# houzhijian/CONE

Measured on AMD Instinct MI355X. Metric: windows/sec + queries/sec, Ego4D-NLQ win_len=90 d=256 top-k=20, higher is better.
Workload: dtype f32

## Files before the change

cone_amd/csrc/api.hip:

```cpp
#include <stdarg.h>
#include <string.h>

#include <vector>

#include "common.h"
#include "gemm_tall.h"
#include "rows_chain.h"

namespace cone {

static thread_local char g_err[512] = "";
void set_error(const char* fmt, ...) {
    va_list ap;
    va_start(ap, fmt);
    vsnprintf(g_err, sizeof(g_err), fmt, ap);
    va_end(ap);
}

struct Linear { const float* w = nullptr; const float* b = nullptr; };
struct LNorm { const float* g = nullptr; const float* b = nullptr; };
struct Mha { const float* in_w = nullptr; const float* in_b = nullptr; Linear out; };
struct EncLayer { Mha sa; Linear l1, l2; LNorm n1, n2; };
struct DecLayer { Mha sa, ca; Linear l1, l2; LNorm n1, n2, n3; };

// ... 13 lines not shown
    const float* txt_pos_emb = nullptr; int txt_pos_rows = 0; cone::LNorm txt_pos_ln;
    int pre_norm = 0; cone::LNorm enc_norm;
    cone::Linear dec_k, dec_v;
    const float* dec_vT[CONE_MAX_LAYERS] = {};
    float* dec0_tgt1 = nullptr; float* dec0_dq = nullptr; float* dec0_scratch = nullptr;
    float* dec_sa_tab[CONE_MAX_LAYERS] = {}; float* dec_ca_tab[CONE_MAX_LAYERS] = {};
    float* tab_arena = nullptr; const float* tab_pos_rows = nullptr; const float* tab_pos_qk = nullptr; int tab_max_v_l = 0;
    int opt_dec_fold = 2;
    int opt_dec0_const = 1;
    int opt_l0_gather = 1;
    int opt_pos_tables = 1;
    int opt_gemm = 0;
    int opt_gemm_tall_min = -1;
    cone::TailWeights enc_tail[CONE_MAX_LAYERS] = {}, dec_tail[CONE_MAX_LAYERS] = {};
    char* split_img = nullptr; char* bf16_img = nullptr;
    int opt_qkv_fused = 1;
    int opt_split_bf16 = 0;
    int opt_bf16 = 0;
    int opt_res_gather = 1;
    int opt_spread = 1;
    int opt_chain = 1;
    int opt_ffn_fused = 2;
    int gen_native = 0;
    int opt_general = 0;
    int opt_general_bf16 = 0;
    char* gen_bf16_img = nullptr;
    struct GenImage { const float* W; const void* img; };
    std::vector<GenImage> gen_bf16_images;
    int opt_max_tokens = CONE_MAX_WINDOW_TOKENS;
    char* f32_img = nullptr; char* f32_tall_img = nullptr;
    struct TallImage { const float* W; int N; const char* img; };
    std::vector<TallImage> tall_images;
    int opt_tail_packed = CONE_TAIL_PACKED_DEFAULT;
    int opt_gemm_tall_packed = CONE_GEMM_TALL_PACKED_DEFAULT;
    const void* tall_image(const float* W, int N) const {
        for (const TallImage& t : tall_images) {
            const uintptr_t w = (uintptr_t)W, base = (uintptr_t)t.W;
            if (w < base || (w - base) % (32 * 256 * sizeof(float)) != 0) continue;
            const size_t off = (w - base) / sizeof(float);
            if (off / 256 + (size_t)N <= (size_t)t.N) return t.img + (size_t)(off / (32 * 256)) * cone::F32_PACK_CHUNK_BYTES;
        }
        return nullptr;
    }
    bool long_windows() const { return opt_max_tokens > CONE_MAX_WINDOW_TOKENS; }
    bool general() const { return gen_native || opt_general || long_windows(); }
};

namespace cone {

struct ArenaBuilder {
    struct Item { const float* src; size_t n; const float** dst; };
    std::vector<Item> items;
    size_t total = 0;
    void add(const float* src, size_t n, const float** dst) {
        items.push_back({src, n, dst});
        total += align_up(n, 64);
    }
};

static int dec0_constants(cone_model* m, hipStream_t s);
static int build_pos_tables(const cone_model* m, int max_v_l, float* pos_rows, float* pos_qk, hipStream_t s);
static int64_t pos_table_rows(int max_v_l) { return (int64_t)max_v_l * (max_v_l + 1) / 2 + 1; }

static void free_model(cone_model* m) {
    if (m->arena) (void)hipFree(m->arena);
    if (m->split_img) (void)hipFree(m->split_img);
// ... 576 lines not shown
                                m->nq, Lmax, s);
    const bool ride = l == 0 && p.sal_ride;
    if (ride) CONE_CHECK_HIP(hipMemsetAsync(c.saliency, 0, (size_t)c.B * c.Lv_max * sizeof(float), s));
    return launch_dec_cross_mfma(f.DQ, XP, MEM, pos, c.vlen, f.off, dl.ca.in_w + 256 * 256, m->dec_vT[l], dl.ca.in_b + 512, f.DATT,
                                 c.B, m->nq, Lmax, l == 0 && p.slabs ? f.QKS : nullptr, s, p.cross[l], ride ? m->saliency.w : nullptr,
                                 ride ? m->saliency.b : nullptr, ride ? c.saliency : nullptr, ride ? c.Lv_max : 0);
}
static AttnSrc table_attn_src(const FwdCall& c, const cone_layer0& l0, int l) {
    const size_t rows = (size_t)pos_table_rows(l0.max_v_l);
    AttnSrc src{};
    src.vlen = c.vlen; src.pos_zero_row = (int)rows - 1;
    src.pos_qk = l0.pos_qk + (size_t)l * rows * 512;
    if (l0.txt_pos_qk) { src.txt_pos_qk = l0.txt_pos_qk + (size_t)l * l0.n_txt * 512; src.trow0 = c.trow0; }
    return src;
}

static int forward_packed_prenorm(const cone_model* m, const FwdCall& c, const FwdPlan& p, FwdBuffers& f, hipStream_t s) {
    const int B = c.B, Lmax = c.Lv_max + c.Lq_max, Mmax = B * Lmax, T = B * m->nq, nd = m->n_dec, ff = m->ff;
    const int* Mdev = f.off + B;
    RUN(launch_scan_lengths(c.vlen, c.qlen, B, f.off, s));
    RUN(launch_pack_pos(c.vproj, c.vrow0, c.vlen, c.tproj, c.trow0, c.qlen, f.off, m->dim_t, f.X, f.POS, f.XP, B, Lmax, s,
                        m->txt_pos_emb, m->txt_pos_ln.g, m->txt_pos_ln.b));
    GemmArgs g;
    for (int l = 0; l < m->n_enc; ++l) {
        const EncLayer& e = m->enc[l];
        RUN(launch_layernorm(f.X, 256, e.n1.g, e.n1.b, f.X1, 256, Mmax, Mdev, 256, s));
        float* QK = f.QKV; float* V = f.QKV + (size_t)Mmax * 512;
        g = G(m, f.X1, 256, e.sa.in_w, 256, e.sa.in_b, QK, 512, Mmax, Mdev, 512, 256);
        g.A2 = f.POS; g.lda2 = 256;
        RUN(launch_gemm(g, s));
        RUN(launch_gemm(G(m, f.X1, 256, e.sa.in_w + 512 * 256, 256, e.sa.in_b + 512, V, 256, Mmax, Mdev, 256, 256), s));
        AttnSrc src{};
        src.Q = QK; src.K = QK + 256; src.V = V; src.ldq = src.ldk = 512; src.ldv = 256;
        RUN(launch_enc_attn(ATTN_PACKED, src, f.ATT, f.off, B, Lmax, s));
        g = G(m, f.ATT, 256, e.sa.out.w, 256, e.sa.out.b, f.X, 256, Mmax, Mdev, 256, 256, EPI_RESIDUAL);
        g.R = f.X; g.ldr = 256;
        RUN(launch_gemm(g, s));
        RUN(launch_layernorm(f.X, 256, e.n2.g, e.n2.b, f.X1, 256, Mmax, Mdev, 256, s));
        RUN(launch_gemm(G(m, f.X1, 256, e.l1.w, 256, e.l1.b, f.H, ff, Mmax, Mdev, ff, 256, EPI_RELU), s));
        g = G(m, f.H, ff, e.l2.w, ff, e.l2.b, f.X, 256, Mmax, Mdev, 256, ff, EPI_RESIDUAL);
        g.R = f.X; g.ldr = 256;
        RUN(launch_gemm(g, s));
    }
    RUN(launch_layernorm(f.X, 256, m->enc_norm.g, m->enc_norm.b, f.X1, 256, Mmax, Mdev, 256, s));
    const float* MEM = f.X1;
    g = G(m, MEM, 256, m->dec_k.w, 256, m->dec_k.b, f.KD, 256 * nd, Mmax, Mdev, 256 * nd, 256);
    g.A2 = f.POS; g.lda2 = 256;
    RUN(launch_gemm(g, s));
    RUN(launch_gemm(G(m, MEM, 256, m->dec_v.w, 256, m->dec_v.b, f.VD, 256 * nd, Mmax, Mdev, 256 * nd, 256), s));
    CONE_CHECK_HIP(hipMemsetAsync(f.TGT, 0, (size_t)T * 256 * sizeof(float), s));
    for (int l = 0; l < nd; ++l) {
        const DecLayer& dl = m->dec[l];
        RUN(dec_layer_front(m, f, l, B, true, s));
        RUN(dec_cross_attn(m, c, p, f, l, MEM, s));
        g = G(m, f.DATT, 256, dl.ca.out.w, 256, dl.ca.out.b, f.TGT, 256, T, nullptr, 256, 256, EPI_RESIDUAL);
        g.R = f.TGT; g.ldr = 256;
        RUN(launch_gemm(g, s));
        RUN(launch_layernorm(f.TGT, 256, dl.n3.g, dl.n3.b, f.TGT1, 256, T, nullptr, 256, s));
        RUN(launch_gemm(G(m, f.TGT1, 256, dl.l1.w, 256, dl.l1.b, f.DH, ff, T, nullptr, ff, 256, EPI_RELU), s));
        g = G(m, f.DH, ff, dl.l2.w, ff, dl.l2.b, f.TGT, 256, T, nullptr, 256, ff, EPI_RESIDUAL);
        g.R = f.TGT; g.ldr = 256;
        RUN(launch_gemm(g, s));
        RUN(launch_layernorm(f.TGT, 256, m->dec_norm.g, m->dec_norm.b, f.HS + (size_t)l * T * 256, 256, T, nullptr, 256, s));
    }
    return heads_and_taps(m, c, HeadBufs{f.HS, f.S1, f.S2, f.LG, f.SP, f.off}, MEM, false, s);
}
// ... 233 lines not shown
        RUN(launch_pack_l0(c.vproj, c.vrow0, c.vlen, c.tproj, c.trow0, c.qlen, f.off, m->dim_t, nullptr, nullptr, nullptr, f.X,
                           nullptr, nullptr, nullptr, B, Lmax, s));
    } else {
        RUN(launch_pack_pos(c.vproj, c.vrow0, c.vlen, c.tproj, c.trow0, c.qlen, f.off, m->dim_t, f.X, f.POS, f.XP, B, Lmax, s,
                            m->txt_pos_emb, m->txt_pos_ln.g, m->txt_pos_ln.b));
    }
    if (p.pre && !p.gather_res)
        RUN(launch_layernorm(f.X, 256, m->enc[0].n1.g, m->enc[0].n1.b, Z, 256, Mmax, Mdev, 256, s));

    bool qkv_fused = false;
    for (int l = 0; l < m->n_enc; ++l) {
        const EncLayer& e = m->enc[l];
        AttnSrc src{};
        int mode = ATTN_PACKED;
        if (l == 0 && p.gather0) {
            mode = ATTN_GATHER;
            src = table_attn_src(c, l0, 0);
            src.qkv_vid = l0.qkv_vid; src.qkv_txt = l0.qkv_txt; src.vrow0 = c.vrow0; src.trow0 = c.trow0;
        } else if (l == 0 && p.caches) {
            src.Q = f.QKV; src.K = f.QKV + 256; src.V = f.QKV + (size_t)Mmax * 512;
            src.ldq = src.ldk = 512; src.ldv = 256;
        } else if (p.tables) {
            if (!qkv_fused)
                RUN(encoder_qkv(m, l, p.pre ? Z : f.X, f.QKV, Mmax, Mdev, s, !p.pre));
            mode = ATTN_POSADD;
            src = table_attn_src(c, l0, l);
            src.Q = f.QKV; src.K = f.QKV + 256; src.V = f.QKV + 512; src.ldq = src.ldk = src.ldv = 768;
        } else {
            float* QK = f.QKV; float* V = f.QKV + (size_t)Mmax * 512;
            RUN(launch_gemm(G(m, f.XP, 256, e.sa.in_w, 256, e.sa.in_b, QK, 512, Mmax, Mdev, 512, 256), s));
            RUN(launch_gemm(G(m, f.X, 256, e.sa.in_w + 512 * 256, 256, e.sa.in_b + 512, V, 256, Mmax, Mdev, 256, 256), s));
            src.Q = QK; src.K = QK + 256; src.V = V; src.ldq = src.ldk = 512; src.ldv = 256;
        }
        RUN(launch_enc_attn(mode, src, f.ATT, f.off, B, Lmax, s));
        const bool g0 = l == 0 && p.gather_res;
        TailArgs t = tail_args(&m->enc_tail[l], f.ATT, g0 ? c.vproj : f.X, f.X, Mmax, Mdev, ff);
        if (g0) { t.r_idx = f.RIDX; t.R2 = c.tproj; }
        if (p.pre) {
            t.pre = true; t.OUT2 = Z; t.ldo2 = 256;
        } else {
            if (l + 1 < m->n_enc) t.next = &m->enc_tail[l + 1];
            t.QKV = f.QKV; t.ldq = 768; t.n_qkv = 768;
            t.X1 = f.X1; t.H = f.H;
            if (!p.tables) { t.C2 = f.XP; t.ADD = f.POS; }
        }
        RUN(launch_layer_tail(m, f, t, s, &qkv_fused));
    }
    const float* MEM = p.pre ? Z : f.X;

    const int h0 = p.h0, HT = (nd - h0) * T;
    const size_t hoff = (size_t)h0 * T;
    float* LGo = p.want_aux ? f.LG + hoff * 2 : c.logits;
    float* SPo = p.want_aux ? f.SP + hoff * 2 : c.spans;
    if (p.dec_xp) RUN(launch_add_pos_rows(MEM, f.off, c.vlen, l0.pos_rows, f.XP, B, Lmax, s, l0.txt_pos, c.trow0));
    if (!p.fold) {
        if (p.dec_tab) RUN(launch_add_pos_rows(MEM, f.off, c.vlen, l0.pos_rows, f.XP, B, Lmax, s));
        GemmArgs g = G(m, f.XP, 256, m->dec_k.w, 256, m->dec_k.b, f.KD, 256 * nd, Mmax, Mdev, 256 * nd, 256);
        RUN(launch_gemm(g, s));
        RUN(launch_gemm(G(m, MEM, 256, m->dec_v.w, 256, m->dec_v.b, f.VD, 256 * nd, Mmax, Mdev, 256 * nd, 256), s));
    }
    if (!p.dec0)
        CONE_CHECK_HIP(hipMemsetAsync(f.TGT, 0, (size_t)T * 256 * sizeof(float), s));
    for (int l = 0; l < nd; ++l) {
        if (l == 0 && p.dec0) RUN(launch_tile_rows2(f.TGT1, m->dec0_tgt1, f.DQ, m->dec0_dq, m->nq, T, s));
        else RUN(dec_layer_front(m, f, l, B, p.pre, s));
        RUN(dec_cross_attn(m, c, p, f, l, MEM, s));
// ... 341 lines not shown
    std::vector<cone_model::GenImage> images;
    char* ip = base;
    int rc = 0;
    for (const Item& it : items) {
        rc = launch_gemm_bf16_pack(it.W, it.K, it.N, it.K, ip, nullptr);
        if (rc) break;
        images.push_back({it.W, ip});
        ip += gemm_bf16_image_bytes(it.N, it.K);
    }
    if (rc == 0 && hipDeviceSynchronize() != hipSuccess) {
        set_error("set_option: general_bf16: building the weight images failed");
        rc = CONE_E_HIP;
    }
    if (rc) { (void)hipFree(base); return rc; }
    m->gen_bf16_img = base;
    m->gen_bf16_images.swap(images);
    return 0;
}

struct OptionRow { const char* name; int cone_model::*field; int lo, hi; bool is_switch; };
static const OptionRow OPTION_ROWS[] = {
    {"dec_fold", &cone_model::opt_dec_fold, 0, 5, false},
    {"l0_gather", &cone_model::opt_l0_gather, 0, 1, true},
    {"dec0_const", &cone_model::opt_dec0_const, 0, 1, true},
    {"pos_tables", &cone_model::opt_pos_tables, 0, 1, true},
    {"ffn_fused", &cone_model::opt_ffn_fused, 0, 2, false},
    {"qkv_fused", &cone_model::opt_qkv_fused, 0, 2, false},
    {"general_shape", &cone_model::opt_general, 0, 1, true},
    {"res_gather", &cone_model::opt_res_gather, 0, 1, true},
    {"rows_chain", &cone_model::opt_chain, 0, 1, true},
    {"ffn_spread", &cone_model::opt_spread, 0, 1, true},
    {"gemm_tall_min_rows", &cone_model::opt_gemm_tall_min, -1, GEMM_TALL_MIN_MAX, false},
    {"tail_packed", &cone_model::opt_tail_packed, 0, 1, true},
};
extern "C" int cone_model_set_option(cone_model* m, const char* name, int value) {
    CONE_REQUIRE(m && name, "set_option: null argument");
    for (const OptionRow& o : OPTION_ROWS) {
        if (strcmp(name, o.name)) continue;
        CONE_REQUIRE(o.is_switch || (value >= o.lo && value <= o.hi), "set_option: %s %d not in [%d, %d]", name, value, o.lo, o.hi);
        m->*o.field = o.is_switch ? value != 0 : value;
        return 0;
    }
    if (!strcmp(name, "max_window_tokens")) {
        CONE_REQUIRE(value >= CONE_MAX_WINDOW_TOKENS && value <= CONE_MAX_LONG_WINDOW_TOKENS,
                     "set_option: max_window_tokens %d not in [%d, %d]", value, CONE_MAX_WINDOW_TOKENS, CONE_MAX_LONG_WINDOW_TOKENS);
        CONE_REQUIRE(value == CONE_MAX_WINDOW_TOKENS || !(m->opt_bf16 || m->opt_split_bf16),
                     "set_option: max_window_tokens %d while bf16 / split_bf16 = 1: windows beyond %d tokens run in exact fp32 "
                     "only (set the mode to 0 first)", value, CONE_MAX_WINDOW_TOKENS);
        m->opt_max_tokens = value;
        return 0;
    }
    const bool split = !strcmp(name, "split_bf16");
    if (split || !strcmp(name, "bf16")) {
        const char* other = split ? "bf16" : "split_bf16";
        CONE_REQUIRE(value == 0 || !m->long_windows(),
                     "set_option: %s on a handle with max_window_tokens = %d: windows beyond %d tokens run the general path, "
                     "exact fp32 only", name, m->opt_max_tokens, CONE_MAX_WINDOW_TOKENS);
        CONE_REQUIRE(value == 0 || (split ? m->split_img : m->bf16_img),
                     "set_option: %s needs hidden_dim 256 with 8 heads and dim_feedforward %% 32 == 0 "
                     "(<= 2048); this handle is hidden_dim %d with %d heads, dim_feedforward %d", name, m->d, m->heads, m->ff);
        CONE_REQUIRE(value == 0 || !(split ? m->opt_bf16 : m->opt_split_bf16),
                     "set_option: %s = 1 while %s = 1: the two modes exclude each other (set %s = 0 first)", name, other, other);
        (split ? m->opt_split_bf16 : m->opt_bf16) = value != 0;
        return 0;
    }
    if (!strcmp(name, "general_bf16")) {
// ... 160 lines not shown
    if (do_pack) {
        const int rc = k.pack(W, nullptr, N, img, (hipStream_t)stream);
        if (rc) return rc;
    }
    return k.rows256(X, 256, img, bias, C, N, M, nullptr, N, (hipStream_t)stream);
}
extern "C" size_t cone_test_proj_split_image_bytes(void) { return TAIL_MODES[TAIL_IMG_SPLIT]->proj_image_bytes(); }
extern "C" int cone_test_proj_ffn_split(const float* A, const float* Wo, const float* bo, const float* R, const float* pg,
                                        const float* pb, const float* W1, const float* b1, const float* W2,
                                        const float* b2, const float* ln_g, const float* ln_b, float* OUT, int M, int ff,
                                        void* img, void* wo_img, int pack, void* stream) {
    bool do_pack;
    const int mode = test_tail_mode(pack, &do_pack);
    const TailMode& k = *TAIL_MODES[mode];
    if (do_pack) {
        int rc = k.pack(W1, W2, ff, img, (hipStream_t)stream);
        if (rc) return rc;
        rc = k.pack(Wo, nullptr, 256, wo_img, (hipStream_t)stream);
        if (rc) return rc;
    }
    TailWeights w;
    const TailArgs t = test_tail(&w, A, Wo, bo, R, pg, pb, W1, b1, W2, b2, ln_g, ln_b, OUT, M, ff);
    w.img[mode] = TailImages{wo_img, img, nullptr};
    return k.proj_ffn(t, (hipStream_t)stream);
}
extern "C" int cone_test_enc_attn(int mode, const float* QKV, const float* qkv_vid, const float* qkv_txt,
                                  const float* pos_qk, const int32_t* vrow0, const int32_t* vlen, const int32_t* trow0,
                                  const int32_t* off, float* OUT, int B, int Lmax, int pos_zero_row, void* stream) {
    AttnSrc a{};
    a.pos_zero_row = pos_zero_row;
    a.Q = QKV; a.K = QKV ? QKV + 256 : nullptr; a.V = QKV ? QKV + 512 : nullptr; a.ldq = a.ldk = a.ldv = 768;
    a.qkv_vid = qkv_vid; a.qkv_txt = qkv_txt; a.pos_qk = pos_qk; a.vrow0 = vrow0; a.vlen = vlen; a.trow0 = trow0;
    a.form = (mode >> 8) & 3;
    return launch_enc_attn(mode & 0xff, a, OUT, off, B, Lmax, (hipStream_t)stream);
}
extern "C" int cone_test_dec_cross(const float* DQ, const float* X, const float* pos_rows, const int32_t* vlen,
                                   const int32_t* off, const float* Wk, const float* WvT, const float* bv, float* OUT,
                                   int B, int nq, int Lmax, int variant, float* qk_slabs, void* stream) {
    if (variant == 1)
        return launch_dec_cross(DQ, nullptr, X, pos_rows, vlen, off, Wk, WvT, bv, OUT, B, nq, Lmax, (hipStream_t)stream);
    return launch_dec_cross_mfma(DQ, nullptr, X, pos_rows, vlen, off, Wk, WvT, bv, OUT, B, nq, Lmax, qk_slabs,
                                 (hipStream_t)stream, variant);
}
extern "C" size_t cone_test_dec_cross_slab_floats(void) { return dec_cross_mfma_slab_floats(); }
extern "C" int cone_test_enc_attn_txt(int mode, const float* QKV, const float* qkv_vid, const float* qkv_txt,
                                      const float* pos_qk, const float* txt_pos_qk, const int32_t* vrow0,
                                      const int32_t* vlen, const int32_t* trow0, const int32_t* off, float* OUT, int B,
                                      int Lmax, int pos_zero_row, void* stream) {
    AttnSrc a{};
    a.pos_zero_row = pos_zero_row;
    a.Q = QKV; a.K = QKV ? QKV + 256 : nullptr; a.V = QKV ? QKV + 512 : nullptr; a.ldq = a.ldk = a.ldv = 768;
    a.qkv_vid = qkv_vid; a.qkv_txt = qkv_txt; a.pos_qk = pos_qk; a.vrow0 = vrow0; a.vlen = vlen; a.trow0 = trow0;
    a.txt_pos_qk = txt_pos_qk;
    a.form = (mode >> 8) & 3;
    return launch_enc_attn(mode & 0xff, a, OUT, off, B, Lmax, (hipStream_t)stream);
}
extern "C" int cone_test_small_attn(const float* Q, int ldq, const float* K, int ldk, const float* V, int ldv, float* OUT,
                                    int ldo, const int32_t* off, int B, int nq, int Lmax, void* stream) {
    return launch_small_attn(Q, ldq, K, ldk, V, ldv, OUT, ldo, off, B, nq, Lmax, (hipStream_t)stream);
}
extern "C" int cone_test_dec_cross_ex(const float* DQ, const float* XP, const float* X, const float* pos_rows,
                                      const int32_t* vlen, const int32_t* off, const float* Wk, const float* WvT,
                                      const float* bv, float* OUT, int B, int nq, int Lmax, int variant, float* qk_slabs,
                                      const float* sal_w, const float* sal_b, float* sal, int sal_ld, void* stream) {
    if (variant == 1) {
        CONE_REQUIRE(!sal, "fused decoder cross-attention: the VALU kernel has no saliency ride");
        return launch_dec_cross(DQ, XP, X, pos_rows, vlen, off, Wk, WvT, bv, OUT, B, nq, Lmax, (hipStream_t)stream);
    }
    return launch_dec_cross_mfma(DQ, XP, X, pos_rows, vlen, off, Wk, WvT, bv, OUT, B, nq, Lmax, qk_slabs, (hipStream_t)stream,
                                 variant, sal_w, sal_b, sal, sal_ld);
}
extern "C" int cone_test_layernorm(const float* x, const float* g, const float* b, float* out, int64_t n_rows,
                                   int dim, void* stream) {
    return launch_layernorm(x, dim, g, b, out, dim, n_rows, nullptr, dim, (hipStream_t)stream);
}
extern "C" int cone_test_gen_attn(const float* Q, int ldq, const float* K, int ldk, const float* V, int ldv, float* OUT, int ldo,
                                  const int32_t* qoff, const int32_t* koff, int B, int nq, int heads, int head_dim, int kcap,
                                  void* stream) {
    return launch_gen_attn(Q, ldq, K, ldk, V, ldv, OUT, ldo, qoff, koff, B, nq, heads, head_dim, kcap, (hipStream_t)stream);
}

extern "C" int cone_test_grid_limit_y(void) { return grid_limit_y(); }
extern "C" int cone_test_scan_lengths(const int32_t* vlen, const int32_t* qlen, int B, int32_t* off, void* stream) {
    return launch_scan_lengths(vlen, qlen, B, off, (hipStream_t)stream);
}
extern "C" int cone_test_compact_index(const int32_t* vlen, const int32_t* voff, int Lv_pad, int32_t* vidx, const int32_t* qlen,
                                       const int32_t* toff, int Lq_pad, int32_t* tidx, int B, void* stream) {
// ... 66 lines not shown
```

cone_amd/csrc/attention.hip:

```cpp
#include "common.h"

#ifndef CONE_ATTN_NT
#define CONE_ATTN_NT 0
#endif

namespace cone {

constexpr float kQScale = 0.17677669529663687f;
constexpr float kQScaleLog2 = 0.17677669529663687f * 1.4426950408889634f;


typedef float f32x4m __attribute__((ext_vector_type(4)));
typedef float f32x2m __attribute__((ext_vector_type(2)));

__device__ __forceinline__ float lane_xor(float v, int lane, int mask) {
    return __int_as_float(__builtin_amdgcn_ds_bpermute((lane ^ mask) << 2, __float_as_int(v)));
}

template <int NKT>
__device__ __forceinline__ float attn_softmax(f32x4m (&sc)[NKT], int L, int lane, int lg) {
    const int lim = L - lg;
    float m = -INFINITY;
#pragma unroll
    for (int kt = 0; kt < NKT; ++kt) {
// ... 2 lines not shown
            for (int r = 0; r < 4; ++r) sc[kt][r] = (16 * kt + 4 * r < lim) ? sc[kt][r] : -INFINITY;
        }
#pragma unroll
        for (int r = 0; r < 4; ++r) m = fmaxf(m, sc[kt][r]);
    }
    m = fmaxf(m, lane_xor(m, lane, 16));
    m = fmaxf(m, lane_xor(m, lane, 32));
    const f32x2m m2 = {m, m};
    f32x2m l2 = {0.f, 0.f};
#pragma unroll
    for (int kt = 0; kt < NKT; ++kt) {
        f32x2m a = sc[kt].xy - m2, b = sc[kt].zw - m2;
        a.x = __builtin_amdgcn_exp2f(a.x); a.y = __builtin_amdgcn_exp2f(a.y);
        b.x = __builtin_amdgcn_exp2f(b.x); b.y = __builtin_amdgcn_exp2f(b.y);
        sc[kt].xy = a; sc[kt].zw = b;
        l2 += a;
        l2 += b;
    }
    float l = l2.x + l2.y;
    l += lane_xor(l, lane, 16);
    l += lane_xor(l, lane, 32);
    return 1.0f / l;
}

__device__ __forceinline__ void attn_normalise(f32x4m& o0, f32x4m& o1, float inv, int lane, int lg) {
#pragma unroll
    for (int r = 0; r < 4; ++r) {
        const float s = __int_as_float(__builtin_amdgcn_ds_bpermute(((lane & 48) + 4 * lg + r) << 2, __float_as_int(inv)));
        o0[r] *= s;
        o1[r] *= s;
    }
}

template <int NKT, int MODE_>
__global__ __launch_bounds__(64 * NKT, (NKT > 12 ? 4 : 6)) void enc_attn16_kernel(AttnSrc a, float* __restrict__ OUT,
                                                                 const int* __restrict__ off) {
    constexpr int MODE = MODE_ & 3;
    constexpr bool TXT = (MODE_ & 4) != 0;
    constexpr int KP = 16 * NKT, LDK = KP + 2, LDV = 36, NT = 64 * NKT;
    constexpr bool DYN = NKT > 12;
    __shared__ float KsT_s[DYN ? 4 : 32 * LDK];
    __shared__ __attribute__((aligned(16))) float Vs_s[DYN ? 4 : KP * LDV];
    extern __shared__ __attribute__((aligned(16))) float attn_dyn[];
    float* const KsT = DYN ? attn_dyn : KsT_s;
    float* const Vs = DYN ? attn_dyn + 32 * LDK : Vs_s;
    const int b = blockIdx.y, head = blockIdx.x;
    const int t0 = off[b];
    const int L = off[b + 1] - t0;
    if (L <= 0) return;
    const int tid = threadIdx.x, lane = tid & 63;
    const int wave = __builtin_amdgcn_readfirstlane(tid >> 6);
    const int li = lane & 15, lg = lane >> 4;
    const unsigned hc = head * 32;
    int lv = 0;
    const float *qb = nullptr, *kb = nullptr, *vb = nullptr, *tb = nullptr, *pb = nullptr;
    unsigned sq = 768, sk = 768, sv = 768;
    int pbase = 0;
    if (MODE != ATTN_PACKED) {
        lv = a.vlen[b];
        pbase = lv * (lv - 1) / 2;
        pb = a.pos_qk + hc;
    }
    if (MODE == ATTN_GATHER) {
        qb = a.qkv_vid + (size_t)a.vrow0[b] * 768 + hc;
        tb = a.qkv_txt + ((ptrdiff_t)a.trow0[b] - lv) * 768 + hc;
    } else {
        sq = a.ldq; sk = a.ldk; sv = a.ldv;
        qb = a.Q + (size_t)t0 * sq + hc; kb = a.K + (size_t)t0 * sk + hc; vb = a.V + (size_t)t0 * sv + hc;
    }
    const int zrow = a.pos_zero_row;
    const float* tpb = nullptr;
    if (TXT) tpb = a.txt_pos_qk + ((ptrdiff_t)a.trow0[b] - lv) * 512 + hc;
    auto prow = [&](int row) -> const float* {
        if (TXT && row >= lv) return tpb + (unsigned)row * 512u;
        return pb + (unsigned)(row < lv ? pbase + row : zrow) * 512u;
    };

    const int q0 = wave * 16;
// ... 3 lines not shown
    {
        const int qrow = min(q0 + li, L - 1);
        const float* qp;
        if (MODE == ATTN_GATHER) qp = (qrow < lv ? qb : tb) + (unsigned)qrow * 768u + 8u * lg;
        else qp = qb + (unsigned)qrow * sq + 8u * lg;
        qx[0] = *reinterpret_cast<const f32x4m*>(qp);
        qx[1] = *reinterpret_cast<const f32x4m*>(qp + 4);
        if (MODE != ATTN_PACKED) {
            const float* pr = prow(qrow) + 8u * lg;
            qt[0] = *reinterpret_cast<const f32x4m*>(pr);
            qt[1] = *reinterpret_cast<const f32x4m*>(pr + 4);
        }
    }
#pragma unroll
    for (int it = 0; it < 2; ++it) {
        const int row = min(kr + it * (NT / 8), L - 1);
        if (MODE == ATTN_GATHER) {
            const float* rp = (row < lv ? qb : tb) + (unsigned)row * 768u + c4;
            kv[it] = *reinterpret_cast<const f32x4m*>(rp + 256);
            vv[it] = *reinterpret_cast<const f32x4m*>(rp + 512);
        } else {
#if CONE_ATTN_NT
            kv[it] = __builtin_nontemporal_load(reinterpret_cast<const f32x4m*>(kb + (unsigned)row * sk + c4));
            vv[it] = __builtin_nontemporal_load(reinterpret_cast<const f32x4m*>(vb + (unsigned)row * sv + c4));
#else
            kv[it] = *reinterpret_cast<const f32x4m*>(kb + (unsigned)row * sk + c4);
            vv[it] = *reinterpret_cast<const f32x4m*>(vb + (unsigned)row * sv + c4);
#endif
        }
        if (MODE != ATTN_PACKED)
            kt_[it] = *reinterpret_cast<const f32x4m*>(prow(row) + 256u + c4);
    }
    float qv[8];
    {
        f32x4m x0 = qx[0], x1 = qx[1];
        if (MODE != ATTN_PACKED) { x0 += qt[0]; x1 += qt[1]; }
        x0 *= kQScaleLog2; x1 *= kQScaleLog2;
#pragma unroll
        for (int j = 0; j < 4; ++j) { qv[j] = x0[j]; qv[4 + j] = x1[j]; }
    }
#pragma unroll
    for (int it = 0; it < 2; ++it) {
        const int key = kr + it * (NT / 8);
        f32x4m k4 = kv[it];
        if (MODE != ATTN_PACKED) k4 += kt_[it];
        const int pos = (key & ~15) + 4 * (key & 3) + ((key >> 2) & 3);
        float* kd = KsT + c4 * LDK + pos;
        kd[0] = k4[0]; kd[LDK] = k4[1]; kd[2 * LDK] = k4[2]; kd[3 * LDK] = k4[3];
        *reinterpret_cast<f32x4m*>(Vs + pos * LDV + c4) = vv[it];
    }
    __syncthreads();
    if (q0 >= L) return;

    f32x4m sc[NKT];
#pragma unroll
    for (int kt = 0; kt < NKT; ++kt) sc[kt] = f32x4m{0.f, 0.f, 0.f, 0.f};
#pragma unroll
    for (int st = 0; st < 8; ++st) {
        const float* kp = KsT + (8 * lg + st) * LDK + li;
#pragma unroll
        for (int kt = 0; kt < NKT; ++kt)
            sc[kt] = __builtin_amdgcn_mfma_f32_16x16x4f32(kp[kt * 16], qv[st], sc[kt], 0, 0, 0);
    }
    const float inv = attn_softmax<NKT>(sc, L, lane, lg);
    f32x4m o0 = {0.f, 0.f, 0.f, 0.f}, o1 = o0;
#pragma unroll
    for (int kt = 0; kt < NKT; ++kt) {
        const float* vp = Vs + (kt * 16 + 4 * lg) * LDV + li;
#pragma unroll
        for (int r = 0; r < 4; ++r) {
            if (kt < NKT - 2 || 16 * kt + 4 * r < L) {
                o0 = __builtin_amdgcn_mfma_f32_16x16x4f32(sc[kt][r], vp[r * LDV], o0, 0, 0, 0);
                o1 = __builtin_amdgcn_mfma_f32_16x16x4f32(sc[kt][r], vp[r * LDV + 16], o1, 0, 0, 0);
            }
        }
    }
    attn_normalise(o0, o1, inv, lane, lg);
    float* ob = OUT + (size_t)t0 * 256 + hc;
    const int qr0 = q0 + 4 * lg;
    const unsigned oo = (unsigned)qr0 * 256u + li;
#pragma unroll
    for (int r = 0; r < 4; ++r) {
        if (qr0 + r < L) {
            ob[oo + 256u * r] = o0[r];
            ob[oo + 256u * r + 16u] = o1[r];
        }
    }
}

template <int NKT, int MODE>
__global__ __launch_bounds__(256, 2) void enc_attn_wave_kernel(AttnSrc a, float* __restrict__ OUT,
                                                               const int* __restrict__ off) {
    const int b = blockIdx.y;
    const int lane = threadIdx.x & 63;
    const int head = blockIdx.x * 4 + __builtin_amdgcn_readfirstlane(threadIdx.x >> 6);
    const int t0 = off[b];
    const int L = off[b + 1] - t0;
    if (L <= 0) return;
    const int li = lane & 15, lg = lane >> 4;
    const unsigned hc = head * 32;
    int lv = 0, pbase = 0;
    const float *qb = nullptr, *kb = nullptr, *vb = nullptr, *tb = nullptr, *pb = nullptr;
    unsigned sq = 768, sk = 768, sv = 768;
    if (MODE != ATTN_PACKED) { lv = a.vlen[b]; pbase = lv * (lv - 1) / 2; pb = a.pos_qk + hc; }
    if (MODE == ATTN_GATHER) {
        qb = a.qkv_vid + (size_t)a.vrow0[b] * 768 + hc;
        tb = a.qkv_txt + ((ptrdiff_t)a.trow0[b] - lv) * 768 + hc;
    } else {
// ... 50 lines not shown
            for (int j = 0; j < 4; ++j) { qv[j] = x0[j]; qv[4 + j] = x1[j]; }
        }
        load_q(q0 + 16 < L ? q0 + 16 : q0);
        f32x4m sc[NKT];
#pragma unroll
        for (int kt = 0; kt < NKT; ++kt) sc[kt] = f32x4m{0.f, 0.f, 0.f, 0.f};
#pragma unroll
        for (int st = 0; st < 8; ++st)
#pragma unroll
            for (int kt = 0; kt < NKT; ++kt)
                sc[kt] = __builtin_amdgcn_mfma_f32_16x16x4f32(kreg[kt][st], qv[st], sc[kt], 0, 0, 0);
        const float inv = attn_softmax<NKT>(sc, L, lane, lg);
        f32x4m o0 = {0.f, 0.f, 0.f, 0.f}, o1 = o0;
#pragma unroll
        for (int kt = 0; kt < NKT; ++kt)
#pragma unroll
            for (int r = 0; r < 4; ++r) {
                o0 = __builtin_amdgcn_mfma_f32_16x16x4f32(sc[kt][r], vreg[kt][r][0], o0, 0, 0, 0);
                o1 = __builtin_amdgcn_mfma_f32_16x16x4f32(sc[kt][r], vreg[kt][r][1], o1, 0, 0, 0);
            }
        attn_normalise(o0, o1, inv, lane, lg);
#pragma unroll
        for (int r = 0; r < 4; ++r) {
            const int qrow = q0 + 4 * lg + r;
            if (qrow < L) {
                float* dst = OUT + (size_t)(t0 + qrow) * 256 + hc + li;
                dst[0] = o0[r];
                dst[16] = o1[r];
            }
        }
    }
}

template <int MODE>
static int launch_enc_attn_t(const AttnSrc& a, float* OUT, const int* off, int B, int Lmax, hipStream_t s) {
    const int nkt = max(6, (Lmax + 15) / 16);
    if (a.form == 2 && nkt <= 9 && !(MODE & 4)) {
        dim3 wgrid(2, B);
#define CONE_ATTNW(N) case N: hipLaunchKernelGGL((enc_attn_wave_kernel<N, (MODE & 3)>), wgrid, dim3(256), 0, s, a, OUT, off); break;
        switch (nkt) { CONE_ATTNW(6) CONE_ATTNW(7) CONE_ATTNW(8) CONE_ATTNW(9) }
#undef CONE_ATTNW
        CONE_LAUNCH_CHECK();
        return 0;
    }
    dim3 grid(8, B);
#define CONE_ATTN16(N) case N: hipLaunchKernelGGL((enc_attn16_kernel<N, MODE>), grid, dim3(64 * N), 0, s, a, OUT, off); break;
#define CONE_ATTN16D(N)                                                                                                     \
    case N: {                                                                                                               \
        constexpr int bytes = (32 * (16 * N + 2) + 16 * N * 36) * 4;                                                        \
        static DeviceOnce once;                                                                                             \
        CONE_CHECK_HIP(device_once(once, [] {                                                                               \
            return hipFuncSetAttribute((const void*)enc_attn16_kernel<N, MODE>, hipFuncAttributeMaxDynamicSharedMemorySize, bytes); \
        }));                                                                                                                \
        hipLaunchKernelGGL((enc_attn16_kernel<N, MODE>), grid, dim3(64 * N), bytes, s, a, OUT, off);                        \
        break;                                                                                                              \
    }
    switch (nkt) {
        CONE_ATTN16(6)
        CONE_ATTN16(7) CONE_ATTN16(8) CONE_ATTN16(9) CONE_ATTN16(10) CONE_ATTN16(11) CONE_ATTN16(12)
        CONE_ATTN16D(13) CONE_ATTN16D(14) CONE_ATTN16D(15) CONE_ATTN16D(16)
    }
#undef CONE_ATTN16
#undef CONE_ATTN16D
    CONE_LAUNCH_CHECK();
    return 0;
}

int launch_enc_attn(int mode, const AttnSrc& a, float* OUT, const int* off, int B, int Lmax, hipStream_t s) {
    CONE_REQUIRE(Lmax >= 1 && Lmax <= 256, "enc attention: window length %d not in [1,256]", Lmax);
    if (B <= 0) return 0;
    ProfScope ps(PK_ENC_ATTN, B, Lmax, mode, nullptr, s);
    switch (mode) {
        case ATTN_PACKED:
            CONE_REQUIRE(a.Q && a.K && a.V, "enc attention: packed mode needs Q, K, V");
            return launch_enc_attn_t<ATTN_PACKED>(a, OUT, off, B, Lmax, s);
        case ATTN_GATHER:
            CONE_REQUIRE(a.qkv_vid && a.qkv_txt && a.pos_qk && a.vrow0 && a.vlen && a.trow0 && a.pos_zero_row >= 0,
                         "enc attention: gather mode needs the layer-0 caches");
            if (a.txt_pos_qk) return launch_enc_attn_t<ATTN_GATHER | 4>(a, OUT, off, B, Lmax, s);
            return launch_enc_attn_t<ATTN_GATHER>(a, OUT, off, B, Lmax, s);
        case ATTN_POSADD:
            CONE_REQUIRE(a.Q && a.K && a.V && a.pos_qk && a.vlen && a.pos_zero_row >= 0,
                         "enc attention: pos-add mode needs Q, K, V, pos_qk, vlen");
            if (a.txt_pos_qk) {
                CONE_REQUIRE(a.trow0, "enc attention: text position rows need trow0");
                return launch_enc_attn_t<ATTN_POSADD | 4>(a, OUT, off, B, Lmax, s);
            }
            return launch_enc_attn_t<ATTN_POSADD>(a, OUT, off, B, Lmax, s);
    }
    set_error("enc attention: unknown mode %d", mode);
    return CONE_E_INVALID;
}

constexpr int kSmallMaxKeys = 192;
template <int MQ>
__global__ __launch_bounds__(64) void small_attn_kernel(const float* __restrict__ Q, int ldq,
                                                        const float* __restrict__ K, int ldk,
                                                        const float* __restrict__ V, int ldv,
                                                        float* __restrict__ OUT, int ldo,
                                                        const int* __restrict__ off, int nq) {
    __shared__ float qs[MQ][32];
    __shared__ float ps[MQ][kSmallMaxKeys];
    const int b = blockIdx.x, head = blockIdx.y, lane = threadIdx.x;
    const int k0 = off ? off[b] : b * nq;
    const int L = off ? off[b + 1] - k0 : nq;
    for (int i = lane; i < nq * 8; i += 64) {
        const int qi = i >> 3, c = i & 7;
        const float4 x = *reinterpret_cast<const float4*>(Q + (size_t)(b * nq + qi) * ldq + head * 32 + c * 4);
        qs[qi][c * 4] = x.x * kQScale; qs[qi][c * 4 + 1] = x.y * kQScale;
        qs[qi][c * 4 + 2] = x.z * kQScale; qs[qi][c * 4 + 3] = x.w * kQScale;
    }
    __syncthreads();
    float sc[3][MQ];
#pragma unroll
    for (int jj = 0; jj < 3; ++jj) {
        const int j = lane + 64 * jj;
#pragma unroll
        for (int qi = 0; qi < MQ; ++qi) sc[jj][qi] = -INFINITY;
        if (j < L) {
            float kv[32];
            const float* kp = K + (size_t)(k0 + j) * ldk + head * 32;
#pragma unroll
// ... 115 lines not shown
```

cone_amd/csrc/common.h:

```cpp
#pragma once
#include <hip/hip_runtime.h>
#include <stdint.h>
#include <stdio.h>

#include <mutex>

#include "../../include/cone_hip.h"

namespace cone {

void set_error(const char* fmt, ...);

#define CONE_CHECK_HIP(expr)                                                                  \
    do {                                                                                      \
        hipError_t _e = (expr);                                                               \
        if (_e != hipSuccess) {                                                               \
            cone::set_error("%s failed: %s (%s:%d)", #expr, hipGetErrorString(_e), __FILE__,  \
                            __LINE__);                                                        \
            return CONE_E_HIP;                                                                \
        }                                                                                     \
    } while (0)

#define CONE_REQUIRE(cond, ...)          \
    do {                                 \
// ... 156 lines not shown
struct TailMode {
    bool (*ffn_supported)(int ff);
    size_t (*ffn_image_bytes)(int ff);
    int (*pack)(const float* W1, const float* W2, int ff, void* img, hipStream_t s);
    int (*ffn)(const float* X, int ldx, const void* Wimg, const float* b1, const float* b2, const float* ln_g, const float* ln_b,
               float* OUT, int ldo, int M, const int* M_dev, int ff, hipStream_t s);
    bool (*rows_supported)(int N);
    size_t (*rows_image_bytes)(int N);
    int (*rows256)(const float* X, int ldx, const void* Wimg, const float* bias, float* C, int ldc, int M, const int* M_dev, int N,
                   hipStream_t s);
    size_t (*proj_image_bytes)();
    bool (*qkv_fits)(int ff, int n_qkv);
    int (*proj_ffn)(const TailArgs& t, hipStream_t s);
    int (*proj_ffn_prenorm)(const TailArgs& t, hipStream_t s);
};
extern const TailMode TAIL_MODE_SPLIT, TAIL_MODE_BF16;

int launch_layernorm(const float* x, int ldx, const float* g, const float* b, float* out, int ldo,
                     int64_t n_rows, const int* n_rows_dev, int dim, hipStream_t s, const int* src_row = nullptr);
int launch_l2norm(const float* x, int64_t n_rows, int dim, float eps, float* out, hipStream_t s, int clamp = 0);
int launch_l2norm_bf16(const float* x, int64_t n_rows, int dim, float eps, uint16_t* out, hipStream_t s, int clamp = 0);
int launch_rows_to_bf16(const float* x, int64_t n_rows, int dim, uint16_t* out, hipStream_t s);
int launch_rowdot(const float* X, int ldx, const float* W, const float* b, float* out, int ldo,
                  int64_t n_rows, int nout, int act, hipStream_t s);

enum { ATTN_PACKED = 0, ATTN_GATHER = 1, ATTN_POSADD = 2 };
struct AttnSrc {
    const float* Q; const float* K; const float* V; int ldq, ldk, ldv;
    const float* qkv_vid; const float* qkv_txt; const float* pos_qk;
    int pos_zero_row;
    const int* vrow0; const int* vlen; const int* trow0;
    const float* txt_pos_qk;
    int form;
};
int launch_enc_attn(int mode, const AttnSrc& src, float* OUT, const int* off, int B, int Lmax, hipStream_t s);
int launch_tile_rows(float* x, int period, int64_t n_rows, hipStream_t s);
int launch_tile_rows2(float* d0, const float* s0, float* d1, const float* s1, int period, int64_t n_rows, hipStream_t s);
bool dec_cross_supported(int nq, int Lmax);
int launch_dec_cross(const float* DQ, const float* XP, const float* X, const float* pos_rows, const int* vlen,
                     const int* off, const float* Wk, const float* WvT, const float* bv, float* OUT, int B, int nq,
                     int Lmax, hipStream_t s);
size_t dec_cross_mfma_slab_floats();
bool dec_cross_mfma_supported(int nq, int Lmax, bool table);
bool dec_cross_res_supported(int nq, int Lmax);
int launch_dec_cross_mfma(const float* DQ, const float* XP, const float* X, const float* pos_rows, const int* vlen,
                          const int* off, const float* Wk, const float* WvT, const float* bv, float* OUT, int B, int nq,
                          int Lmax, float* qk_slabs, hipStream_t s, int form = 2, const float* sal_w = nullptr,
                          const float* sal_b = nullptr, float* sal = nullptr, int sal_ld = 0);
int launch_small_attn(const float* Q, int ldq, const float* K, int ldk, const float* V, int ldv, float* OUT,
                      int ldo, const int* off, int B, int nq, int Lmax, hipStream_t s);

int launch_scan_lengths(const int* vlen, const int* qlen , int B, int* off, hipStream_t s);
int launch_compact_index(const int* vlen, const int* voff, int Lv_pad, int* vidx, const int* qlen, const int* toff, int Lq_pad,
                         int* tidx, int B, hipStream_t s);
int launch_pack_pos(const float* vproj, const int* vrow0, const int* vlen, const float* tproj, const int* trow0,
                    const int* qlen, const int* off, const float* dim_t, float* X, float* POS, float* XP, int B,
                    int Lmax, hipStream_t s, const float* tpe = nullptr, const float* tpg = nullptr,
                    const float* tpb = nullptr);
int launch_pos_rows(const float* dim_t, int max_v_l, float* out, hipStream_t s);
int launch_add_pos_rows(const float* MEM, const int* off, const int* vlen, const float* pos_rows, float* XP, int B, int Lmax,
                        hipStream_t s, const float* txt_pos = nullptr, const int* trow0 = nullptr);
int launch_txt_pos_rows(const float* tproj, const int* tok_index, const int* src_row, int mod, int n_emb, const float* tpe,
                        const float* tpg, const float* tpb, int n, const int* n_dev, float* out, hipStream_t s);
int launch_row_index(const int* vrow0, const int* vlen, const int* trow0, const int* qlen, const int* off, int* ridx,
                     int B, int Lmax, hipStream_t s);
int launch_pack_l0(const float* vproj, const int* vrow0, const int* vlen, const float* tproj, const int* trow0,
                   const int* qlen, const int* off, const float* dim_t, const float* qkv_vid, const float* qkv_txt,
// ... 24 lines not shown
```

Before: 383,300.

## Add swizzled LDS layout with double-buffered vector fetches in encoder attention

Adds a FETCH variant of the encoder attention kernel. In it, K is stored row-major in LDS with an XOR swizzle and V is stored transposed with a conflict-free stride, so each lane reads 16-byte vectors instead of scalar loads. The QK and PV MFMA loops are software-pipelined: the next tile's LDS reads are issued before the counted lgkmcnt wait, with sched barriers to keep that order. This targets LDS read latency and bank conflicts in the attention inner loops. It is on by default, with an option to fall back, and it adds register pressure and hand-scheduling risk.

```diff
diff --git a/cone_amd/csrc/api.hip b/cone_amd/csrc/api.hip
--- a/cone_amd/csrc/api.hip
+++ b/cone_amd/csrc/api.hip
@@ -69,6 +69,7 @@
     struct TallImage { const float* W; int N; const char* img; };
     std::vector<TallImage> tall_images;
     int opt_tail_packed = CONE_TAIL_PACKED_DEFAULT;
+    int opt_attn_fetch = CONE_ATTN_FETCH_DEFAULT;
     int opt_gemm_tall_packed = CONE_GEMM_TALL_PACKED_DEFAULT;
     const void* tall_image(const float* W, int N) const {
         for (const TallImage& t : tall_images) {
@@ -711,6 +712,7 @@
         RUN(launch_gemm(G(m, f.X1, 256, e.sa.in_w + 512 * 256, 256, e.sa.in_b + 512, V, 256, Mmax, Mdev, 256, 256), s));
         AttnSrc src{};
         src.Q = QK; src.K = QK + 256; src.V = V; src.ldq = src.ldk = 512; src.ldv = 256;
+        src.fetch = m->opt_attn_fetch ? 2 : 1;
         RUN(launch_enc_attn(ATTN_PACKED, src, f.ATT, f.off, B, Lmax, s));
         g = G(m, f.ATT, 256, e.sa.out.w, 256, e.sa.out.b, f.X, 256, Mmax, Mdev, 256, 256, EPI_RESIDUAL);
         g.R = f.X; g.ldr = 256;
@@ -1010,6 +1012,7 @@
             RUN(launch_gemm(G(m, f.X, 256, e.sa.in_w + 512 * 256, 256, e.sa.in_b + 512, V, 256, Mmax, Mdev, 256, 256), s));
             src.Q = QK; src.K = QK + 256; src.V = V; src.ldq = src.ldk = 512; src.ldv = 256;
         }
+        src.fetch = m->opt_attn_fetch ? 2 : 1;
         RUN(launch_enc_attn(mode, src, f.ATT, f.off, B, Lmax, s));
         const bool g0 = l == 0 && p.gather_res;
         TailArgs t = tail_args(&m->enc_tail[l], f.ATT, g0 ? c.vproj : f.X, f.X, Mmax, Mdev, ff);
@@ -1417,6 +1420,7 @@
     {"ffn_spread", &cone_model::opt_spread, 0, 1, true},
     {"gemm_tall_min_rows", &cone_model::opt_gemm_tall_min, -1, GEMM_TALL_MIN_MAX, false},
     {"tail_packed", &cone_model::opt_tail_packed, 0, 1, true},
+    {"attn_fetch", &cone_model::opt_attn_fetch, 0, 1, true},
 };
 extern "C" int cone_model_set_option(cone_model* m, const char* name, int value) {
     CONE_REQUIRE(m && name, "set_option: null argument");
@@ -1643,6 +1647,7 @@
     a.Q = QKV; a.K = QKV ? QKV + 256 : nullptr; a.V = QKV ? QKV + 512 : nullptr; a.ldq = a.ldk = a.ldv = 768;
     a.qkv_vid = qkv_vid; a.qkv_txt = qkv_txt; a.pos_qk = pos_qk; a.vrow0 = vrow0; a.vlen = vlen; a.trow0 = trow0;
     a.form = (mode >> 8) & 3;
+    a.fetch = (mode >> 10) & 3;
     return launch_enc_attn(mode & 0xff, a, OUT, off, B, Lmax, (hipStream_t)stream);
 }
 extern "C" int cone_test_dec_cross(const float* DQ, const float* X, const float* pos_rows, const int32_t* vlen,
@@ -1664,6 +1669,7 @@
     a.qkv_vid = qkv_vid; a.qkv_txt = qkv_txt; a.pos_qk = pos_qk; a.vrow0 = vrow0; a.vlen = vlen; a.trow0 = trow0;
     a.txt_pos_qk = txt_pos_qk;
     a.form = (mode >> 8) & 3;
+    a.fetch = (mode >> 10) & 3;
     return launch_enc_attn(mode & 0xff, a, OUT, off, B, Lmax, (hipStream_t)stream);
 }
 extern "C" int cone_test_small_attn(const float* Q, int ldq, const float* K, int ldk, const float* V, int ldv, float* OUT,
diff --git a/cone_amd/csrc/attention.hip b/cone_amd/csrc/attention.hip
--- a/cone_amd/csrc/attention.hip
+++ b/cone_amd/csrc/attention.hip
@@ -58,18 +58,34 @@
     }
 }
 
-template <int NKT, int MODE_>
+constexpr int ATTN_FETCH_READS = 2;
+constexpr int attn_ldvt(int nkt) { return (16 * nkt + 59) / 64 * 64 + 4; }
+constexpr int attn_lds_floats(int nkt, bool fetch) {
+    return fetch ? 16 * nkt * 32 + 32 * attn_ldvt(nkt) : 32 * (16 * nkt + 2) + 16 * nkt * 36;
+}
+#define ATTN_SB() __builtin_amdgcn_sched_barrier(0)
+template <int N>
+__device__ __forceinline__ void attn_lgkm_wait() {
+    ATTN_SB();
+    asm volatile("s_waitcnt lgkmcnt(%0)" ::"n"(N) : "memory");
+    ATTN_SB();
+}
+
+template <int NKT, int MODE_, bool FETCH>
 __global__ __launch_bounds__(64 * NKT, (NKT > 12 ? 4 : 6)) void enc_attn16_kernel(AttnSrc a, float* __restrict__ OUT,
                                                                  const int* __restrict__ off) {
     constexpr int MODE = MODE_ & 3;
     constexpr bool TXT = (MODE_ & 4) != 0;
-    constexpr int KP = 16 * NKT, LDK = KP + 2, LDV = 36, NT = 64 * NKT;
+    constexpr int KP = 16 * NKT, LDK = FETCH ? 32 : KP + 2, LDV = FETCH ? attn_ldvt(NKT) : 36, NT = 64 * NKT;
+    constexpr int KFL = FETCH ? KP * LDK : 32 * LDK, VFL = FETCH ? 32 * LDV : KP * LDV;
+    static_assert(KFL + VFL == attn_lds_floats(NKT, FETCH), "the launcher requests what the images take");
+    static_assert(!FETCH || (LDV >= KP && LDV % 4 == 0 && (LDV / 4) % 16 == 1), "V image: 16-B columns, conflict-free stride");
     constexpr bool DYN = NKT > 12;
-    __shared__ float KsT_s[DYN ? 4 : 32 * LDK];
-    __shared__ __attribute__((aligned(16))) float Vs_s[DYN ? 4 : KP * LDV];
+    __shared__ __attribute__((aligned(16))) float KsT_s[DYN ? 4 : KFL];
+    __shared__ __attribute__((aligned(16))) float Vs_s[DYN ? 4 : VFL];
     extern __shared__ __attribute__((aligned(16))) float attn_dyn[];
     float* const KsT = DYN ? attn_dyn : KsT_s;
-    float* const Vs = DYN ? attn_dyn + 32 * LDK : Vs_s;
+    float* const Vs = DYN ? attn_dyn + KFL : Vs_s;
     const int b = blockIdx.y, head = blockIdx.x;
     const int t0 = off[b];
     const int L = off[b + 1] - t0;
@@ -139,22 +155,29 @@
             kt_[it] = *reinterpret_cast<const f32x4m*>(prow(row) + 256u + c4);
     }
     float qv[8];
-    {
+    auto scale_q = [&] {
         f32x4m x0 = qx[0], x1 = qx[1];
         if (MODE != ATTN_PACKED) { x0 += qt[0]; x1 += qt[1]; }
         x0 *= kQScaleLog2; x1 *= kQScaleLog2;
 #pragma unroll
         for (int j = 0; j < 4; ++j) { qv[j] = x0[j]; qv[4 + j] = x1[j]; }
-    }
+    };
+    if (!FETCH) scale_q();
 #pragma unroll
     for (int it = 0; it < 2; ++it) {
         const int key = kr + it * (NT / 8);
         f32x4m k4 = kv[it];
         if (MODE != ATTN_PACKED) k4 += kt_[it];
         const int pos = (key & ~15) + 4 * (key & 3) + ((key >> 2) & 3);
-        float* kd = KsT + c4 * LDK + pos;
-        kd[0] = k4[0]; kd[LDK] = k4[1]; kd[2 * LDK] = k4[2]; kd[3 * LDK] = k4[3];
-        *reinterpret_cast<f32x4m*>(Vs + pos * LDV + c4) = vv[it];
+        if (FETCH) {
+            *reinterpret_cast<f32x4m*>(KsT + pos * LDK + (c4 ^ ((pos << 1) & 20))) = k4;
+            float* vd = Vs + c4 * LDV + pos;
+            vd[0] = vv[it][0]; vd[LDV] = vv[it][1]; vd[2 * LDV] = vv[it][2]; vd[3 * LDV] = vv[it][3];
+        } else {
+            float* kd = KsT + c4 * LDK + pos;
+            kd[0] = k4[0]; kd[LDK] = k4[1]; kd[2 * LDK] = k4[2]; kd[3 * LDK] = k4[3];
+            *reinterpret_cast<f32x4m*>(Vs + pos * LDV + c4) = vv[it];
+        }
     }
     __syncthreads();
     if (q0 >= L) return;
@@ -162,6 +185,52 @@
     f32x4m sc[NKT];
 #pragma unroll
     for (int kt = 0; kt < NKT; ++kt) sc[kt] = f32x4m{0.f, 0.f, 0.f, 0.f};
+    f32x4m o0 = {0.f, 0.f, 0.f, 0.f}, o1 = o0;
+    float inv;
+    if (FETCH) {
+        f32x4m kf[2][ATTN_FETCH_READS], vf[2][ATTN_FETCH_READS];
+        static_assert(sizeof(kf[0]) == 16 * ATTN_FETCH_READS && sizeof(vf[0]) == 16 * ATTN_FETCH_READS,
+                      "the counted wait leaves exactly the next tile's reads in flight");
+        const int sw = (li >> 1) & 5;
+        const f32x4m* ka = reinterpret_cast<const f32x4m*>(KsT + li * LDK + (((2 * lg) ^ sw) << 2));
+        const f32x4m* kb = reinterpret_cast<const f32x4m*>(KsT + li * LDK + (((2 * lg + 1) ^ sw) << 2));
+        const f32x4m* va = reinterpret_cast<const f32x4m*>(Vs + li * LDV + 4 * lg);
+        kf[0][0] = ka[0]; kf[0][1] = kb[0];
+        ATTN_SB();
+        scale_q();
+#pragma unroll
+        for (int kt = 0; kt < NKT; ++kt) {
+            if (kt + 1 < NKT) {
+                kf[(kt + 1) & 1][0] = ka[(kt + 1) * 4 * LDK]; kf[(kt + 1) & 1][1] = kb[(kt + 1) * 4 * LDK];
+                attn_lgkm_wait<ATTN_FETCH_READS>();
+            } else {
+                vf[0][0] = va[0]; vf[0][1] = va[4 * LDV];
+                attn_lgkm_wait<ATTN_FETCH_READS>();
+            }
+#pragma unroll
+            for (int st = 0; st < 8; ++st)
+                sc[kt] = __builtin_amdgcn_mfma_f32_16x16x4f32(kf[kt & 1][st >> 2][st & 3], qv[st], sc[kt], 0, 0, 0);
+            ATTN_SB();
+        }
+        inv = attn_softmax<NKT>(sc, L, lane, lg);
+#pragma unroll
+        for (int kt = 0; kt < NKT; ++kt) {
+            if (kt + 1 < NKT) {
+                vf[(kt + 1) & 1][0] = va[(kt + 1) * 4]; vf[(kt + 1) & 1][1] = va[(kt + 1) * 4 + 4 * LDV];
+                attn_lgkm_wait<ATTN_FETCH_READS>();
+            } else {
+                attn_lgkm_wait<0>();
+            }
+#pragma unroll
+            for (int r = 0; r < 4; ++r) {
+                if (kt < NKT - 2 || 16 * kt + 4 * r < L) {
+                    o0 = __builtin_amdgcn_mfma_f32_16x16x4f32(sc[kt][r], vf[kt & 1][0][r], o0, 0, 0, 0);
+                    o1 = __builtin_amdgcn_mfma_f32_16x16x4f32(sc[kt][r], vf[kt & 1][1][r], o1, 0, 0, 0);
+                }
+            }
+            ATTN_SB();
+        }
+    } else {
 #pragma unroll
     for (int st = 0; st < 8; ++st) {
         const float* kp = KsT + (8 * lg + st) * LDK + li;
@@ -169,8 +238,7 @@
         for (int kt = 0; kt < NKT; ++kt)
             sc[kt] = __builtin_amdgcn_mfma_f32_16x16x4f32(kp[kt * 16], qv[st], sc[kt], 0, 0, 0);
     }
-    const float inv = attn_softmax<NKT>(sc, L, lane, lg);
-    f32x4m o0 = {0.f, 0.f, 0.f, 0.f}, o1 = o0;
+    inv = attn_softmax<NKT>(sc, L, lane, lg);
 #pragma unroll
     for (int kt = 0; kt < NKT; ++kt) {
         const float* vp = Vs + (kt * 16 + 4 * lg) * LDV + li;
@@ -181,6 +249,7 @@
                 o1 = __builtin_amdgcn_mfma_f32_16x16x4f32(sc[kt][r], vp[r * LDV + 16], o1, 0, 0, 0);
             }
         }
+    }
     }
     attn_normalise(o0, o1, inv, lane, lg);
     float* ob = OUT + (size_t)t0 * 256 + hc;
@@ -297,7 +366,7 @@
     }
 }
 
-template <int MODE>
+template <int MODE, bool FETCH>
 static int launch_enc_attn_t(const AttnSrc& a, float* OUT, const int* off, int B, int Lmax, hipStream_t s) {
     const int nkt = max(6, (Lmax + 15) / 16);
     if (a.form == 2 && nkt <= 9 && !(MODE & 4)) {
@@ -309,15 +378,15 @@
         return 0;
     }
     dim3 grid(8, B);
-#define CONE_ATTN16(N) case N: hipLaunchKernelGGL((enc_attn16_kernel<N, MODE>), grid, dim3(64 * N), 0, s, a, OUT, off); break;
+#define CONE_ATTN16(N) case N: hipLaunchKernelGGL((enc_attn16_kernel<N, MODE, FETCH>), grid, dim3(64 * N), 0, s, a, OUT, off); break;
 #define CONE_ATTN16D(N)                                                                                                     \
     case N: {                                                                                                               \
-        constexpr int bytes = (32 * (16 * N + 2) + 16 * N * 36) * 4;                                                        \
+        constexpr int bytes = attn_lds_floats(N, FETCH) * 4;                                                                \
         static DeviceOnce once;                                                                                             \
         CONE_CHECK_HIP(device_once(once, [] {                                                                               \
-            return hipFuncSetAttribute((const void*)enc_attn16_kernel<N, MODE>, hipFuncAttributeMaxDynamicSharedMemorySize, bytes); \
+            return hipFuncSetAttribute((const void*)enc_attn16_kernel<N, MODE, FETCH>, hipFuncAttributeMaxDynamicSharedMemorySize, bytes); \
         }));                                                                                                                \
-        hipLaunchKernelGGL((enc_attn16_kernel<N, MODE>), grid, dim3(64 * N), bytes, s, a, OUT, off);                        \
+        hipLaunchKernelGGL((enc_attn16_kernel<N, MODE, FETCH>), grid, dim3(64 * N), bytes, s, a, OUT, off);                 \
         break;                                                                                                              \
     }
     switch (nkt) {
@@ -335,24 +404,27 @@
     CONE_REQUIRE(Lmax >= 1 && Lmax <= 256, "enc attention: window length %d not in [1,256]", Lmax);
     if (B <= 0) return 0;
     ProfScope ps(PK_ENC_ATTN, B, Lmax, mode, nullptr, s);
+    const bool fetch = a.fetch ? a.fetch == 2 : CONE_ATTN_FETCH_DEFAULT != 0;
+#define CONE_ATTN_T(M) (fetch ? launch_enc_attn_t<(M), true>(a, OUT, off, B, Lmax, s) : launch_enc_attn_t<(M), false>(a, OUT, off, B, Lmax, s))
     switch (mode) {
         case ATTN_PACKED:
             CONE_REQUIRE(a.Q && a.K && a.V, "enc attention: packed mode needs Q, K, V");
-            return launch_enc_attn_t<ATTN_PACKED>(a, OUT, off, B, Lmax, s);
+            return CONE_ATTN_T(ATTN_PACKED);
         case ATTN_GATHER:
             CONE_REQUIRE(a.qkv_vid && a.qkv_txt && a.pos_qk && a.vrow0 && a.vlen && a.trow0 && a.pos_zero_row >= 0,
                          "enc attention: gather mode needs the layer-0 caches");
-            if (a.txt_pos_qk) return launch_enc_attn_t<ATTN_GATHER | 4>(a, OUT, off, B, Lmax, s);
-            return launch_enc_attn_t<ATTN_GATHER>(a, OUT, off, B, Lmax, s);
+            if (a.txt_pos_qk) return CONE_ATTN_T(ATTN_GATHER | 4);
+            return CONE_ATTN_T(ATTN_GATHER);
         case ATTN_POSADD:
             CONE_REQUIRE(a.Q && a.K && a.V && a.pos_qk && a.vlen && a.pos_zero_row >= 0,
                          "enc attention: pos-add mode needs Q, K, V, pos_qk, vlen");
             if (a.txt_pos_qk) {
                 CONE_REQUIRE(a.trow0, "enc attention: text position rows need trow0");
-                return launch_enc_attn_t<ATTN_POSADD | 4>(a, OUT, off, B, Lmax, s);
-            }
-            return launch_enc_attn_t<ATTN_POSADD>(a, OUT, off, B, Lmax, s);
-    }
+                return CONE_ATTN_T(ATTN_POSADD | 4);
+            }
+            return CONE_ATTN_T(ATTN_POSADD);
+    }
+#undef CONE_ATTN_T
     set_error("enc attention: unknown mode %d", mode);
     return CONE_E_INVALID;
 }
diff --git a/cone_amd/csrc/common.h b/cone_amd/csrc/common.h
--- a/cone_amd/csrc/common.h
+++ b/cone_amd/csrc/common.h
@@ -212,7 +212,11 @@
     const int* vrow0; const int* vlen; const int* trow0;
     const float* txt_pos_qk;
     int form;
-};
+    int fetch;
+};
+#ifndef CONE_ATTN_FETCH_DEFAULT
+#define CONE_ATTN_FETCH_DEFAULT 1
+#endif
 int launch_enc_attn(int mode, const AttnSrc& src, float* OUT, const int* off, int B, int Lmax, hipStream_t s);
 int launch_tile_rows(float* x, int period, int64_t n_rows, hipStream_t s);
 int launch_tile_rows2(float* d0, const float* s0, float* d1, const float* s1, int period, int64_t n_rows, hipStream_t s);
```

New measurement: 382,700, median of 2. Within noise of the previous version (-0.1%).
